# facebookresearch/DetectAndTrack

Measured on AMD Instinct MI355X. Metric: clips/sec (8-frame 800px), higher is better.
Workload: dtype bf16; 1 GPU; 3D R-18 FPN3D keypoint R-CNN inference, 4 clip(s) of 1x3x8x768x1344 per step (= per forward) per GPU (kT=3 body+FPN, slice-center 2D heads, per clip: 1000 proposals, 100 detections -> kps_score -> decoded keypoints); mode=infer, weights=random-init (synthetic_params, seed 3), images_per_forward=4, forwards_in_flight=3, clips_in_flight=12, keyframe_dce=False, hip_graph=True, resident_input=True, parallelism=clip-sharded x1 (no data-path collective)

## Files before the change

### detectandtrack_amd/csrc/conv_special.hip

```cpp
#include "conv_internal.h"

using namespace dat_conv;

namespace {

struct Ws64Params {
    const char* x;
    const char* w;
    const float* scale;
    const float* bias;
    const char* res;
    char* y;
    const char* zeros;
    int frames, H, W, out_cs, relu, res_mode;
    int tiles_h, tiles_w, ntiles;
    int ablate;
};

template <int TWL>
__global__ __launch_bounds__(NTHREADS) __attribute__((amdgpu_waves_per_eu(1, 1))) void conv3x3_c64_ws_kernel(const Ws64Params p) {
    constexpr int TW = 1 << TWL, TH = 256 >> TWL, PW = TW + 2, PH = TH + 2;
    constexpr int NPIX = PH * PW, NPIECE = (NPIX * 8 + 63) / 64, PBYTES = NPIECE * 1024, UMAX = (NPIECE + 3) / 4;
    extern __shared__ __attribute__((aligned(16))) char smem[];
    const int tid = threadIdx.x, lane = tid & 63;
// ... 598 lines not shown
__global__ __launch_bounds__(KS_THREADS) void conv_kt1x1_ks_kernel(const TkParams p) {
    constexpr int CB = 256;
    constexpr int NWQ = CB / 64;
    constexpr int NJ = NWQ;
    constexpr int WBYTES = CB / 32 * 4 * 1024;
    constexpr int WPIECES = CB / 64;
    extern __shared__ __attribute__((aligned(16))) char smem[];
    char* const xb = smem;
    char* const wb = smem + 3 * KS_XBYTES;
    const int tid = threadIdx.x, lane = tid & 63;
    const int wave = __builtin_amdgcn_readfirstlane(tid >> 6);
    const int khalf = lane >> 5, n = lane & 31;
    unsigned bid = blockIdx.x;
    if (p.xcd) bid = xcd_block_map(bid, gridDim.x);
    const int cb = bid % p.ncb;
    const unsigned pos0 = (bid / p.ncb) * 256u;
    const int wq = wave % NWQ, ph = wave / NWQ;
    typedef const __attribute__((address_space(1))) void* gptr_t;
    typedef __attribute__((address_space(3))) void* lptr_t;
    const char* xsrc[4];
    int tq[4];
#pragma unroll
    for (int u = 0; u < 4; ++u) {
        const int row = wave * 32 + u * 8 + (lane >> 3);
        const int slot = (lane & 7) ^ ((row >> 1) & 7);
        const unsigned pos = min(pos0 + (unsigned)row, p.npos - 1u);
        const unsigned f = pos / p.how;
        tq[u] = (int)(f % (unsigned)p.T);
        xsrc[u] = p.x + (size_t)pos * (unsigned)p.in_cs * 2u + slot * 16;
    }
    const char* wsrc = p.w + (size_t)cb * (CB / 32) * 4096 + (size_t)(wave * WPIECES) * 1024 + lane * 16;
    const size_t wstep = (size_t)p.mb_total * 4096;
    const ptrdiff_t fstep = (ptrdiff_t)p.how * p.in_cs * 2;
    char* const xdma = xb + wave * (32 * 128);
    char* const wdma = wb + wave * (WPIECES * 1024);
    int rq_t = 0, rq_c = 0;
#define TK_DMA_X(BUF_)                                                                                       \
    {                                                                                                        \
        const int kt_ = min(rq_t, p.kt_n - 1), cc_ = rq_t < p.kt_n ? rq_c : p.ncc - 1;                       \
        const int dt_ = kt_ - p.pt;                                                                          \
        const ptrdiff_t off_ = (ptrdiff_t)dt_ * fstep + cc_ * 128;                                           \
        _Pragma("unroll") for (int u_ = 0; u_ < 4; ++u_) {                                                   \
            const bool in_ = (unsigned)(tq[u_] + dt_) < (unsigned)p.T;                                       \
            const char* s_ = in_ ? xsrc[u_] + off_ : p.zeros;                                     \
            __builtin_amdgcn_global_load_lds((gptr_t)s_, (lptr_t)(xdma + (BUF_) * KS_XBYTES + u_ * 1024), 16, 0, 0); \
        }                                                                                                    \
        if (++rq_c == p.ncc) { rq_c = 0; ++rq_t; }                                                           \
    }
#define TK_DMA_W(KC_, BUF_)                                                                                  \
    {                                                                                                        \
        const char* ws_ = wsrc + (size_t)min((KC_), p.kchunks - 1) * wstep;                                  \
        _Pragma("unroll") for (int u_ = 0; u_ < WPIECES; ++u_)                                               \
            __builtin_amdgcn_global_load_lds((gptr_t)(ws_ + u_ * 1024), (lptr_t)(wdma + (BUF_) * WBYTES + u_ * 1024), 16, 0, 0); \
    }
#define TK_COMPUTE(XBUF_, WBUF_)                                                                             \
    {                                                                                                        \
        const char* xc_ = xb + (XBUF_) * KS_XBYTES + b_base;                                                 \
        const char* wc_ = wb + (WBUF_) * WBYTES + a_off;                                                     \
        _Pragma("unroll") for (int ks_ = 0; ks_ < 4; ++ks_) {                                                \
            uint4 a_[2], b_[NJ];                                                                             \
            _Pragma("unroll") for (int i_ = 0; i_ < 2; ++i_) a_[i_] = *(const uint4*)(wc_ + (i_ * 4 + ks_) * 1024); \
            _Pragma("unroll") for (int j_ = 0; j_ < NJ; ++j_) b_[j_] = *(const uint4*)(xc_ + j_ * 4096 + b_slot[ks_]); \
            _Pragma("unroll") for (int i_ = 0; i_ < 2; ++i_)                                                 \
                _Pragma("unroll") for (int j_ = 0; j_ < NJ; ++j_) Mma<DAT_BF16>::step(a_[i_], b_[j_], acc[i_][j_]); \
        }                                                                                                    \
    }
    TK_DMA_W(0, 0);
    TK_DMA_X(0);
    TK_DMA_X(1);
    f32x16_t acc[2][NJ];
#pragma unroll
    for (int i = 0; i < 2; ++i)
#pragma unroll
        for (int j = 0; j < NJ; ++j)
#pragma unroll
            for (int r = 0; r < 16; ++r) acc[i][j][r] = 0.f;
    const int a_off = (2 * wq) * 4096 + lane * 16;
    const int b_base = (ph * (32 * NJ) + n) * 128;
    int b_slot[4];
#pragma unroll
    for (int ks = 0; ks < 4; ++ks) b_slot[ks] = (((ks * 2 + khalf) ^ (n >> 1)) & 7) << 4;
    asm volatile("s_waitcnt vmcnt(4)" ::: "memory");
    __syncthreads();
    int xi = 0;
    for (int kc = 0; kc < p.kchunks; ++kc) {
        const int x2 = xi >= 1 ? xi - 1 : 2;
        TK_DMA_W(kc + 1, (kc + 1) & 1);
        TK_DMA_X(x2);
        TK_COMPUTE(xi, kc & 1);
        asm volatile("s_waitcnt vmcnt(4)" ::: "memory");
        __syncthreads();
        xi = xi == 2 ? 0 : xi + 1;
    }
    asm volatile("s_waitcnt vmcnt(0)" ::: "memory");
    __syncthreads();
#undef TK_DMA_X
#undef TK_DMA_W
#undef TK_COMPUTE
    char* const est = smem + wave * (32 * EPI_PITCH);
    const int sq = lane & 7, spl = lane >> 3;
    const int c0 = cb * CB + wq * 64 + sq * 8;
    float sc[8], bi[8];
#pragma unroll
    for (int e = 0; e < 8; ++e) {
        const bool ok = c0 + e < p.cout;
        const int c = ok ? c0 + e : 0;
        sc[e] = ok ? (p.scale ? p.scale[c] : 1.f) : 0.f;
        bi[e] = (ok && p.bias) ? p.bias[c] : 0.f;
    }
    const unsigned cres = (unsigned)min(c0, p.out_cs - 8);
#pragma unroll
    for (int j = 0; j < NJ; ++j) {
        const unsigned tile0 = pos0 + (unsigned)(ph * (32 * NJ) + j * 32);
        uint4 rr[4];
        if (p.res_mode) {
#pragma unroll
            for (int r = 0; r < 4; ++r) {
                const unsigned pc = min(tile0 + (unsigned)(r * 8 + spl), p.npos - 1u);
                rr[r] = *(const uint4*)(p.res + ((size_t)pc * (unsigned)p.out_cs + cres) * 2u);
            }
        }
#pragma unroll
        for (int i = 0; i < 2; ++i) epi_stage(est, n, khalf, i, acc[i][j]);
        __builtin_amdgcn_wave_barrier();
#pragma unroll
        for (int r = 0; r < 4; ++r) {
            const int pl = r * 8 + spl;
            float v[8];
            epi_load(est, pl, sq * 8, v);
            epi_affine(v, sc, bi);
            if (p.res_mode) epi_residual<DAT_BF16>(v, rr[r], 1);
            epi_relu(v, p.relu);
            const unsigned pos = tile0 + (unsigned)pl;
            if (pos < p.npos && c0 < p.cout)
                epi_store<DAT_BF16>(p.y + ((size_t)pos * (unsigned)p.out_cs + (unsigned)c0) * 2u, v);
        }
        __builtin_amdgcn_wave_barrier();
    }
}

template <int TWL, int R, int MF>
__global__ __launch_bounds__(NTHREADS) __attribute__((amdgpu_waves_per_eu(1, 1))) void conv3x3_bt_kernel(const ConvParams p) {
    constexpr int TW = 1 << TWL, TH = 256 >> TWL, PW = TW + 2, PH = TH + 2;
    constexpr int NPIX = PH * PW, NPIECE = (NPIX * 8 + 63) / 64, PBYTES = NPIECE * 1024, UMAX = (NPIECE + 3) / 4;
    constexpr int NSTEP = MF ? 18 : 36, APS = MF ? 8 : 4;
    static_assert(NSTEP % R == 0 && PBYTES < 65536, "ring slots are static per unrolled step; 16-bit patch addresses");
    static_assert(APS * R + UMAX < 64, "vmcnt is a 6-bit counter");
    typedef unsigned u32x4_t __attribute__((ext_vector_type(4)));
    typedef const __attribute__((address_space(1))) void* gptr_t;
    typedef __attribute__((address_space(3))) void* lptr_t;
    extern __shared__ __attribute__((aligned(16))) char smem[];
    unsigned long long clk_c0 = 0, clk_r0 = 0;
    if (p.clk) { clk_c0 = __builtin_amdgcn_s_memtime(); clk_r0 = __builtin_amdgcn_s_memrealtime(); }
    const int tid = threadIdx.x, lane = tid & 63;
    const int wave = __builtin_amdgcn_readfirstlane(tid >> 6);
    const int wave_n = wave & 1, wave_p = wave >> 1;
    const int khalf = lane >> 5, n = lane & 31;

    const unsigned bid = xcd_block_map(blockIdx.x, p.nblocks);
    const int nb = bid % p.nblk_n;
    unsigned tile = bid / p.nblk_n;
    const int fc = tile % p.otn; tile /= p.otn;
    const int tw_i = tile % p.tiles_w; tile /= p.tiles_w;
    const int th_i = tile % p.tiles_h;
    const int clip = tile / p.tiles_h;
    const int f = clip * p.otn + fc;
    const int t = p.ot0 + fc;
    const int f_in = clip * p.T + t;
    const int oh0 = th_i * TH, ow0 = tw_i * TW;

    int kt_lo = 0, kt_hi = p.KT - 1;
    while (kt_lo < p.KT && (t + kt_lo - p.pt) < p.in_lo) ++kt_lo;
    while (kt_hi >= 0 && (t + kt_hi - p.pt) >= p.in_hi) --kt_hi;
    const int n_kt = kt_hi - kt_lo + 1;
    const int npat = n_kt * p.n_cchunks;
    const int kt_hi_x = kt_lo + n_kt;
    int kshift = 0;
    if (n_kt == p.KT && (DAT_KT_ROTATE)) kshift = (p.KT - (t + kt_lo - p.pt) % p.KT) % p.KT;
    int kt = kt_lo + kshift, cc = 0;
    if (kt >= kt_hi_x) kt -= n_kt;

    constexpr int NJ = MF ? 8 : 4;
    unsigned qp[9][NJ / 2];
#pragma unroll
    for (int tp = 0; tp < 9; ++tp)
#pragma unroll
        for (int j = 0; j < NJ; ++j) {
            const int pos = wave_p * 128 + (MF ? j * 16 + (lane & 15) : j * 32 + n);
            const int r = pos >> TWL, c = pos & (TW - 1);
            const int row = (r + tp / 3) * PW + c + tp % 3;
            const unsigned a16 = patch_frag_addr<MF>(row, MF ? lane >> 4 : khalf);
            if (j & 1) qp[tp][j >> 1] |= a16 << 16; else qp[tp][j >> 1] = a16;
        }
    const size_t wd_cc_stride = (size_t)(p.Cout_pad >> 5) * 4096;
    const size_t tap_stride = (size_t)p.n_cchunks * wd_cc_stride;
    const char* const wd_base = p.w + (size_t)(nb * 8 + wave_n * 4) * 4096;
    unsigned aoff[APS];
#pragma unroll
    for (int i = 0; i < APS; ++i) {
        if (MF) {
            const unsigned kg = (unsigned)lane >> 4;
            aoff[i] = 16u * ((unsigned)((i & 1) << 4) + ((unsigned)lane & 15u) + 32u * (kg & 1u)) + (kg >> 1) * 1024u + (unsigned)(i >> 1) * 4096u;
        } else {
            aoff[i] = (unsigned)lane * 16u + (unsigned)i * 4096u;
        }
    }

#define BT_DMA(KT_, CC_, B_)                                                                                              \
    {                                                                                                                     \
        const int fin_ = f_in + (KT_) - p.pt;                                                                             \
        const char* xf_ = p.x + ((size_t)fin_ * p.H * p.W) * p.Cin * 2 + (size_t)(CC_) * 128;                             \
        _Pragma("unroll") for (int u_ = 0; u_ < UMAX; ++u_) {                                                             \
            const int piece_ = min(wave + 4 * u_, NPIECE - 1);                                                            \
            const int it_ = piece_ * 64 + lane, row_ = it_ >> 3;                                                          \
            const int slot_ = patch_src_slot<MF>(it_);                                                                    \
            const int prow_ = row_ / PW, pcol_ = row_ - prow_ * PW;                                                       \
            const int ih_ = oh0 - 1 + prow_, iw_ = ow0 - 1 + pcol_;                                                       \
            const bool ok_ = row_ < NPIX && (unsigned)ih_ < (unsigned)p.H && (unsigned)iw_ < (unsigned)p.W;               \
            const char* src_ = ok_ ? xf_ + ((size_t)(unsigned)(ih_ * p.W + iw_) * (unsigned)(p.Cin * 2) + (unsigned)(slot_ * 16)) : p.zeros; \
            __builtin_amdgcn_global_load_lds((gptr_t)src_, (lptr_t)(smem + (B_) * PBYTES + piece_ * 1024), 16, 0, 0);     \
        }                                                                                                                 \
    }
#define BT_WPATCH(KT_, CC_) (wd_base + ((size_t)((KT_) * 9) * p.n_cchunks + (CC_)) * wd_cc_stride)
    constexpr int SPT = NSTEP / 9;
#define BT_ALOAD(WP_, S_, SLOT_)                                                                                          \
    {                                                                                                                     \
        const char* wt_ = (WP_) + (size_t)((S_) / SPT) * tap_stride;                                                      \
        _Pragma("unroll") for (int i_ = 0; i_ < APS; ++i_)                                                                \
            asm volatile("global_load_dwordx4 %0, %1, %2 offset:%3" : "=v"(aq[SLOT_][i_]) : "v"(aoff[i_]), "s"(wt_), "n"(((S_) % SPT) * (4096 / SPT)) : "memory"); \
    }
#define BT_BREAD(U_, BOFF_)                                                                                               \
    {                                                                                                                     \
        if ((U_) % 4 == 0) {                                                                                              \
            unsigned q0_ = qp[(U_) / 4][0], q1_ = qp[(U_) / 4][1], q2_ = qp[(U_) / 4][NJ / 2 - 2], q3_ = qp[(U_) / 4][NJ / 2 - 1]; \
            asm volatile("" : "+v"(q0_), "+v"(q1_));    \
            ba[0] = (q0_ & 0xffffu) + (BOFF_); ba[1] = (q0_ >> 16) + (BOFF_);                                             \
            ba[2] = (q1_ & 0xffffu) + (BOFF_); ba[3] = (q1_ >> 16) + (BOFF_);                                             \
            if constexpr (MF != 0) {                                                                                      \
                asm volatile("" : "+v"(q2_), "+v"(q3_));                                                                  \
                ba[NJ - 4] = (q2_ & 0xffffu) + (BOFF_); ba[NJ - 3] = (q2_ >> 16) + (BOFF_);                               \
                ba[NJ - 2] = (q3_ & 0xffffu) + (BOFF_); ba[NJ - 1] = (q3_ >> 16) + (BOFF_);                               \
            }                                                                                                             \
        }                                                                                                                 \
        _Pragma("unroll") for (int j_ = 0; j_ < 4; ++j_)                                                                  \
            asm volatile("ds_read_b128 %0, %1" : "=v"(bq[(U_) % 2][j_])                                                   \
                         : "v"(ba[(MF ? ((U_) % 2) * 4 : 0) + j_] ^ (unsigned)(MF ? (((U_) / 2) % 2) << 6 : ((U_) % 4) << 5)) : "memory"); \
    }
#define BT_MFMA(ACC_, A_, B_)                                                                                             \
    {                                                                                                                     \
        if constexpr (MF) asm volatile(DAT_MFMA16K32_OP " %0, %1, %2, %0" : "+a"(ACC_) : "v"(A_), "v"(B_) : "memory");    \
        else asm volatile(DAT_MFMA16_OP " %0, %1, %2, %0" : "+a"(ACC_) : "v"(A_), "v"(B_) : "memory");                    \
    }

    typedef std::conditional_t<MF != 0, f32x4_t, f32x16_t> acc_t;
    acc_t acc[APS][NJ];
#pragma unroll
    for (int i = 0; i < APS; ++i)
#pragma unroll
        for (int j = 0; j < NJ; ++j)
#pragma unroll
            for (int r = 0; r < (MF ? 4 : 16); ++r) acc[i][j][r] = 0.f;
    u32x4_t aq[R][APS], bq[2][4];
    unsigned ba[NJ] = {};

    if (npat > 0) {
        BT_DMA(kt, cc, 0);
        const char* wcur = BT_WPATCH(kt, cc);
        static_for(std::make_integer_sequence<int, R>{}, [&](auto ic_) __attribute__((always_inline)) {
            constexpr int s0 = decltype(ic_)::value;
            (void)&aq; (void)&aoff;
            BT_ALOAD(wcur, s0, s0);
        });
        asm volatile("s_waitcnt vmcnt(%0)" :: "n"(APS * R) : "memory");
        __syncthreads();
        int buf = 0;
        for (int pi = 0; pi < npat; ++pi, buf ^= 1) {
            int ncc = cc + 1, nkt = kt;
            if (ncc == p.n_cchunks) { ncc = 0; if (++nkt == kt_hi_x) nkt = kt_lo; }
            const bool has_next = pi + 1 < npat;
            if (has_next) BT_DMA(nkt, ncc, buf ^ 1);
            const char* wnxt = has_next ? BT_WPATCH(nkt, ncc) : wcur;
            const unsigned boff = (unsigned)buf * PBYTES;
            __builtin_amdgcn_s_setprio(1);
            BT_BREAD(0, boff);
            static_for(std::make_integer_sequence<int, 36>{}, [&](auto ic_) __attribute__((always_inline)) {
                constexpr int un = decltype(ic_)::value;
                constexpr int st = MF ? un / 2 : un, jb = MF ? (un % 2) * 4 : 0;
                constexpr bool opens = !MF || un % 2 == 0, ends = !MF || un % 2 == 1;
                (void)&aq; (void)&aoff; (void)&bq; (void)&ba; (void)&acc; (void)&qp;
                if (un + 1 < 36) BT_BREAD(un + 1, boff);
                if (un + 1 < 36) asm volatile("s_waitcnt lgkmcnt(4)" ::: "memory"); else asm volatile("s_waitcnt lgkmcnt(0)" ::: "memory");
                if constexpr (opens) {
                    if constexpr (st < R) {
                        if (has_next) asm volatile("s_waitcnt vmcnt(%0)" :: "n"(APS * (R - 1) + UMAX) : "memory");
                        else asm volatile("s_waitcnt vmcnt(%0)" :: "n"(APS * (R - 1)) : "memory");
                    } else {
                        asm volatile("s_waitcnt vmcnt(%0)" :: "n"(APS * (R - 1)) : "memory");
                    }
                }
#pragma unroll
                for (int i = 0; i < APS; ++i)
#pragma unroll
                    for (int j = 0; j < 4; ++j) BT_MFMA(acc[i][jb + j], aq[st % R][i], bq[un % 2][j]);
                if constexpr (ends) {
                    if constexpr (st + R < NSTEP) { BT_ALOAD(wcur, st + R, st % R); } else { BT_ALOAD(wnxt, st + R - NSTEP, st % R); }
                }
            });
            __builtin_amdgcn_s_setprio(0);
            __syncthreads();
            kt = nkt; cc = ncc; wcur = wnxt;
        }
    }
    asm volatile("s_waitcnt vmcnt(0) lgkmcnt(0)\n\ts_nop 15\n\ts_nop 15" ::: "memory");
#undef BT_MFMA
#undef BT_BREAD
#undef BT_ALOAD
#undef BT_WPATCH
#undef BT_DMA

    constexpr int EPITCH = EPI_PITCH;
    char* const est = smem + wave * (32 * EPITCH);
    const int sl_c = (lane & 7) * 8, sl_p = lane >> 3;
    const size_t tile_pos = ((size_t)f * p.Ho + oh0) * p.Wo + ow0;
    char* const ybase = p.y + tile_pos * p.out_cs * 2;
    const char* const rbase = p.res_mode == 2 ? p.res + (size_t)f * (p.Ho >> 1) * (p.Wo >> 1) * p.out_cs * 2 : p.res + tile_pos * p.out_cs * 2;
#pragma unroll
    for (int h = 0; h < 2; ++h) {
        const int c_st = nb * 256 + wave_n * 128 + h * 64 + sl_c;
        float sc[8], bi[8];
#pragma unroll
        for (int e = 0; e < 8; ++e) {
            const bool ok = (c_st + e) < p.Cout;
            sc[e] = (p.scale && ok) ? p.scale[c_st + e] : 1.f;
            bi[e] = (p.bias && ok) ? p.bias[c_st + e] : 0.f;
        }
        uint4 rq[2][4];
        const bool res_on = p.res_mode && c_st < p.Cout;
        auto res_fetch = [&](int j, uint4* dst) __attribute__((always_inline)) {
#pragma unroll
            for (int q = 0; q < 4; ++q) {
                const int pl = q * 8 + sl_p;
                const int ohl = TWL == 5 ? 4 * wave_p + j : 8 * wave_p + 2 * j + (pl >> 4), owl = TWL == 5 ? pl : (pl & 15);
                const int oh = oh0 + ohl, ow = ow0 + owl;
                const bool live = oh < p.Ho && ow < p.Wo && !(p.ablate & 4);
                unsigned rpos = (unsigned)(ohl * p.Wo + owl);
                if (p.res_mode == 2) rpos = (unsigned)((oh >> 1) * (p.Wo >> 1) + (ow >> 1));
                dst[q] = *(const uint4*)(rbase + (live ? (rpos * (unsigned)p.out_cs + (unsigned)c_st) * 2u : 0u));
            }
        };
        if (res_on) res_fetch(0, rq[0]);
#pragma unroll
        for (int j = 0; j < 4; ++j) {
            if (res_on && j + 1 < 4) res_fetch(j + 1, rq[(j + 1) & 1]);
            if constexpr (MF) {
#pragma unroll
                for (int i = 0; i < 4; ++i)
#pragma unroll
                    for (int jl = 0; jl < 2; ++jl) epi_stage16(est, lane, i, jl, acc[(4 * h + i) % APS][(2 * j + jl) % NJ]);
            } else {
#pragma unroll
                for (int i = 0; i < 2; ++i)
#pragma unroll
                    for (int g = 0; g < 4; ++g)
                        *(float4*)(est + n * EPITCH + (i * 32 + g * 8 + khalf * 4) * 4) =
                            make_float4(acc[2 * h + i][j][g * 4 + 0], acc[2 * h + i][j][g * 4 + 1], acc[2 * h + i][j][g * 4 + 2], acc[2 * h + i][j][g * 4 + 3]);
            }
            __builtin_amdgcn_wave_barrier();
#pragma unroll
            for (int q = 0; q < 4; ++q) {
                const int pl = q * 8 + sl_p;
                const float4 t0 = *(const float4*)(est + pl * EPITCH + sl_c * 4);
                const float4 t1 = *(const float4*)(est + pl * EPITCH + sl_c * 4 + 16);
                float v[8] = {t0.x, t0.y, t0.z, t0.w, t1.x, t1.y, t1.z, t1.w};
                const int ohl = TWL == 5 ? 4 * wave_p + j : 8 * wave_p + 2 * j + (pl >> 4), owl = TWL == 5 ? pl : (pl & 15);
                const int oh = oh0 + ohl, ow = ow0 + owl;
                if (oh >= p.Ho || ow >= p.Wo || c_st >= p.Cout || (p.ablate & 4)) continue;
                const unsigned lpos = (unsigned)(ohl * p.Wo + owl);
#pragma unroll
                for (int e = 0; e < 8; ++e) v[e] = v[e] * sc[e] + bi[e];
                if (p.res_mode) {
                    const uint4 r = rq[j & 1][q];
                    const uint32_t ru[4] = {r.x, r.y, r.z, r.w};
#pragma unroll
                    for (int e2 = 0; e2 < 4; ++e2) {
                        v[2 * e2] += bf2f((uint16_t)(ru[e2] & 0xffff));
                        v[2 * e2 + 1] += bf2f((uint16_t)(ru[e2] >> 16));
                    }
                }
                if (p.relu) {
#pragma unroll
                    for (int e = 0; e < 8; ++e) v[e] = fmaxf(v[e], 0.f);
                }
                *(uint4*)(ybase + (lpos * (unsigned)p.out_cs + (unsigned)c_st) * 2u) =
                    make_uint4(f2bf2(v[0], v[1]), f2bf2(v[2], v[3]), f2bf2(v[4], v[5]), f2bf2(v[6], v[7]));
            }
            __builtin_amdgcn_wave_barrier();
        }
    }
    if (p.clk && threadIdx.x == 0) {
        atomicAdd(&p.clk[0], __builtin_amdgcn_s_memtime() - clk_c0);
        atomicAdd(&p.clk[1], __builtin_amdgcn_s_memrealtime() - clk_r0);
    }
}

}

namespace dat_conv {

bool ws64_eligible(const dat_ctx* ctx, const dat_conv_desc* d) {
    return ctx->dbg_ws64 && d->dtype == DAT_BF16 && d->Cin == 64 && d->Cout == 64 && d->KT == 1 && d->KH == 3 && d->KW == 3 &&
           d->stride_h == 1 && d->stride_w == 1 && d->pad_h == 1 && d->pad_w == 1 && d->pad_t == 0 && d->res_mode != 2 &&
           d->out_tn <= 0 && d->out_cstride % 8 == 0 && conv_dilation(d) == 1;
}

int ctx_num_cu(dat_ctx* ctx);
static long long persist_cus(dat_ctx* ctx, int mult) {
    long long n = ctx_num_cu(ctx);
    if (ctx->dbg_persist_pct > 0 && ctx->dbg_persist_pct < 100) n = std::max<long long>(mult, n * ctx->dbg_persist_pct / 100 / mult * mult);
    return n;
}

int ctx_num_cu(dat_ctx* ctx) {
    if (ctx->num_cu == 0) {
        int dev = 0, n = 0;
        if (hipGetDevice(&dev) != hipSuccess || hipDeviceGetAttribute(&n, hipDeviceAttributeMultiprocessorCount, dev) != hipSuccess) n = 0;
        ctx->num_cu = n > 0 ? n : 256;
    }
    return ctx->num_cu;
}

bool bt_eligible(const dat_ctx* ctx, const dat_conv_desc* d) {
    return ctx->dbg_bt && d->dtype == DAT_BF16 && d->Cin % 64 == 0 && cout_pad_of(d) % 256 == 0 && d->Cout % 8 == 0 && d->KH == 3 && d->KW == 3 &&
           d->stride_h == 1 && d->stride_w == 1 && d->pad_h == 1 && d->pad_w == 1 && d->out_cstride % 8 == 0 && conv_dilation(d) == 1;
}

int bt_tile_twl(const ConvParams& p, long long* nblocks) {
    int best = 4;
    long long best_tiles = -1;
    for (int twl = 4; twl <= 5; ++twl) {
        const long long tiles = cdiv_ll(p.Ho, 256 >> twl) * cdiv_ll(p.Wo, 1 << twl);
        if (best_tiles < 0 || tiles < best_tiles) { best_tiles = tiles; best = twl; }
    }
    *nblocks = best_tiles * p.frames * (p.Cout_pad / 256);
    return best;
}

int launch_bt(dat_ctx* ctx, hipStream_t st, ConvParams& p) {
    long long nblocks = 0;
    const int twl = bt_tile_twl(p, &nblocks);
    const int tw = 1 << twl, th = 256 >> twl;
    p.th_log2 = 8 - twl; p.tw_log2 = twl; p.tile_w = tw;
    p.tiles_h = (int)cdiv_ll(p.Ho, th); p.tiles_w = (int)cdiv_ll(p.Wo, tw);
    p.n_cchunks = p.Cin / 64;
    p.nblk_n = p.Cout_pad / 256;
    p.ksplit = 1; p.part = nullptr;
    p.ablate = ctx->dbg_ablate;
    DAT_ENFORCE(ctx, nblocks > 0 && nblocks < (1ll << 31), "conv3d: grid of %lld blocks unsupported", nblocks);
    DAT_ENFORCE(ctx, (long long)p.Ho * p.Wo * std::max(p.out_cs, p.Cout) * 4 < (1ll << 31) && (long long)p.H * p.W * p.Cin * 2 < (1ll << 32),
                "conv3d: one frame of %dx%d exceeds the 32-bit offsets of the big-tile kernel", p.H, p.W);
    p.nblocks = (unsigned)nblocks;
    const int npiece = ((th + 2) * (tw + 2) * 8 + 63) / 64;
    const size_t lds = (size_t)2 * npiece * 1024;
#define BT_LAUNCH(TWL_, R_, MF_)                                                                                           \
    {                                                                                                                  \
        if (dat_ensure_lds(ctx, (const void*)conv3x3_bt_kernel<TWL_, R_, MF_>, 160 * 1024) != DAT_OK) return DAT_ERR_LAUNCH; \
        hipLaunchKernelGGL((conv3x3_bt_kernel<TWL_, R_, MF_>), dim3(p.nblocks), dim3(NTHREADS), lds, st, p);           \
    }
    if (ctx->dbg_mfma) { if (twl == 5) BT_LAUNCH(5, 3, 1) else BT_LAUNCH(4, 3, 1) }
    else if (twl == 5) BT_LAUNCH(5, 6, 0) else BT_LAUNCH(4, 6, 0)
#undef BT_LAUNCH
    DAT_CHECK_LAUNCH(ctx, "conv3x3_bt");
    return DAT_OK;
}

bool pw256_eligible(const dat_ctx* ctx, const dat_conv_desc* d) {
    return ctx->dbg_ws64 && d->dtype == DAT_BF16 && d->Cin == 64 && d->Cout == 256 && d->KT == 1 && d->KH == 1 && d->KW == 1 &&
           d->stride_h == 1 && d->stride_w == 1 && d->pad_h == 0 && d->pad_w == 0 && d->pad_t == 0 && d->out_tn <= 0 &&
           d->out_cstride % 8 == 0 &&
           (long long)d->H * d->W >= 32 && (long long)d->H * d->W * d->W < (1ll << 32) &&
           (long long)d->frames * d->H * d->W * std::max(d->out_cstride, 64) * 2 < (1ll << 32);
}

int launch_pw256(dat_ctx* ctx, hipStream_t st, const ConvParams& cp) {
    Pw256Params p;
    p.x = cp.x; p.w = cp.w; p.scale = cp.scale; p.bias = cp.bias; p.res = cp.res; p.y = cp.y;
    p.npos = (long long)cp.frames * cp.H * cp.W;
    p.H = cp.H; p.W = cp.W; p.out_cs = cp.out_cs; p.relu = cp.relu; p.res_mode = cp.res_mode;
    const long long ntiles = cdiv_ll(p.npos, 32);
    DAT_ENFORCE(ctx, ntiles > 0 && ntiles < (1ll << 31), "conv3d: %lld wave tiles unsupported", ntiles);
    p.ntiles = (int)ntiles;
    p.hw = (unsigned)(cp.H * cp.W);
    p.w_magic = cp.W == 1 ? 0u : (unsigned)((0x100000000ull + (unsigned)cp.W - 1) / (unsigned)cp.W);
    const unsigned grid = (unsigned)std::min<long long>(cdiv_ll(ntiles, 4), persist_cus(ctx, 8));
    const size_t lds = (size_t)4 * 32 * (256 * 4 + 16);
    if (dat_ensure_lds(ctx, (const void*)conv1x1_k64_c256_ws_kernel, 160 * 1024) != DAT_OK) return DAT_ERR_LAUNCH;
    hipLaunchKernelGGL(conv1x1_k64_c256_ws_kernel, dim3(grid), dim3(NTHREADS), lds, st, p);
    DAT_CHECK_LAUNCH(ctx, "conv1x1_k64_c256_ws");
    return DAT_OK;
}

static int lw_nsplit(const dat_conv_desc* d) {
    const long long wbytes = (long long)d->Cin * cout_pad_of(d) * 2;
    int ns = 1;
    while (wbytes / ns > 128 * 1024) ns *= 2;
    return ns;
}

bool pwlw_eligible(dat_ctx* ctx, const dat_conv_desc* d) {
    if (!(ctx->dbg_pwlw && d->dtype == DAT_BF16 && d->KT == 1 && d->KH == 1 && d->KW == 1 && d->pad_h == 0 && d->pad_w == 0 && d->pad_t == 0 &&
          d->out_tn <= 0 && d->stride_h == d->stride_w && (d->stride_h == 1 || d->stride_h == 2)))
        return false;
    const int kc = d->Cin / 64;
    if (d->Cin % 64 || !(kc == 1 || kc == 2 || kc == 4 || kc == 8)) return false;
    const int ns = lw_nsplit(d), mbt = cout_pad_of(d) / 32;
    if (ns > 4 || mbt % ns) return false;
    const int mbp = mbt / ns;
    if (!(mbp == 2 || mbp == 4 || mbp == 8 || mbp == 16) || (kc == 8 && mbp > 4)) return false;
    if ((long long)kc * mbp * 4096 + mbp * 256 + 4 * 32 * 144 > 160 * 1024) return false;
    if (d->out_cstride % 8 || d->out_cstride < d->Cout) return false;
    int Ho, Wo;
    dat_conv3d_out_shape(d, &Ho, &Wo);
    const long long npos = (long long)d->frames * Ho * Wo;
    if ((long long)Ho * Wo < 32 || (long long)Ho * Wo * Wo >= (1ll << 32)) return false;
    if (npos >= (1ll << 31) || (long long)d->frames * d->H * d->W >= (1ll << 31)) return false;
    return npos / 32 >= 2ll * 4 * ctx_num_cu(ctx) / ns;
}

template <int KC, int MBW, int NPASS>
static int launch_pwlw_t(dat_ctx* ctx, hipStream_t st, const PwLwParams& p, unsigned grid, size_t lds) {
    if (p.res_mode == 4) {
        if (dat_ensure_lds(ctx, (const void*)conv1x1_lw_kernel<KC, MBW, NPASS, 1>, 160 * 1024) != DAT_OK) return DAT_ERR_LAUNCH;
        hipLaunchKernelGGL((conv1x1_lw_kernel<KC, MBW, NPASS, 1>), dim3(grid), dim3(NTHREADS), lds, st, p);
        return DAT_OK;
    }
    if (dat_ensure_lds(ctx, (const void*)conv1x1_lw_kernel<KC, MBW, NPASS>, 160 * 1024) != DAT_OK) return DAT_ERR_LAUNCH;
    hipLaunchKernelGGL((conv1x1_lw_kernel<KC, MBW, NPASS>), dim3(grid), dim3(NTHREADS), lds, st, p);
    return DAT_OK;
}

int launch_pwlw(dat_ctx* ctx, hipStream_t st, const ConvParams& cp, const dat_conv_desc* d) {
    PwLwParams p;
    p.x = cp.x; p.w = cp.w; p.scale = cp.scale; p.bias = cp.bias; p.res = cp.res; p.y = cp.y; p.res2 = cp.res2;
    p.npos = (unsigned)((long long)cp.frames * cp.Ho * cp.Wo);
    p.Ho = cp.Ho; p.Wo = cp.Wo; p.H = cp.H; p.W = cp.W; p.stride = cp.sh;
    p.in_cs = cp.Cin; p.out_cs = cp.out_cs; p.cout = cp.Cout; p.relu = cp.relu; p.res_mode = cp.res_mode;
    p.ntiles = (int)cdiv_ll(p.npos, 32);
    p.how = (unsigned)(cp.Ho * cp.Wo);
    p.wo_magic = cp.Wo == 1 ? 0u : (unsigned)((0x100000000ull + (unsigned)cp.Wo - 1) / (unsigned)cp.Wo);
    p.nsplit = lw_nsplit(d); p.mb_total = cp.Cout_pad / 32;
    const int kc = cp.Cin / 64, mbp = p.mb_total / p.nsplit;
    const int mbw = kc <= 4 ? std::min(mbp, 8) : std::min(mbp, 4), npass = mbp / mbw;
    const long long per_part = std::min<long long>(cdiv_ll(p.ntiles, 4), persist_cus(ctx, 8 * p.nsplit) / p.nsplit);
    const unsigned grid = (unsigned)(per_part * p.nsplit);
    p.xcd = ctx->dbg_pw_xcd && p.nsplit > 1 && grid % (8u * (unsigned)p.nsplit) == 0;
    const size_t lds = (size_t)kc * mbp * 4096 + (size_t)mbp * 32 * 8 + 4 * 32 * (32 * 4 + 16);
    DAT_ENFORCE(ctx, lds <= 160 * 1024, "conv1x1_lw: %zu bytes of LDS", lds);
    int rc = DAT_ERR_UNSUPPORTED;
#define LW_CASE(KC_, MBW_, NP_) if (kc == KC_ && mbw == MBW_ && npass == NP_) rc = launch_pwlw_t<KC_, MBW_, NP_>(ctx, st, p, grid, lds);
    LW_CASE(1, 2, 1) LW_CASE(1, 4, 1) LW_CASE(1, 8, 1) LW_CASE(1, 8, 2)
    LW_CASE(2, 2, 1) LW_CASE(2, 4, 1) LW_CASE(2, 8, 1) LW_CASE(2, 8, 2)
    LW_CASE(4, 2, 1) LW_CASE(4, 4, 1) LW_CASE(4, 8, 1)
    LW_CASE(8, 2, 1) LW_CASE(8, 4, 1)
#undef LW_CASE
    if (rc != DAT_OK) DAT_FAIL(ctx, rc, "conv1x1_lw: no instantiation for K chunks %d x %d row blocks x %d passes", kc, mbw, npass);
    DAT_CHECK_LAUNCH(ctx, "conv1x1_lw");
    return DAT_OK;
}

bool pwks_eligible(dat_ctx* ctx, const dat_conv_desc* d) {
    if (!(ctx->dbg_pwks > 0 && d->dtype == DAT_BF16 && d->KT == 1 && d->KH == 1 && d->KW == 1 && d->pad_h == 0 && d->pad_w == 0 && d->pad_t == 0 &&
          d->out_tn <= 0 && d->stride_h == d->stride_w && (d->stride_h == 1 || d->stride_h == 2)))
        return false;
    if (d->Cin % 64 || d->Cin / 64 < ctx->dbg_pwks || cout_pad_of(d) % 256) return false;
    if (d->out_cstride % 8 || d->out_cstride < d->Cout || d->out_cstride < 8) return false;
    int Ho, Wo;
    dat_conv3d_out_shape(d, &Ho, &Wo);
    const long long npos = (long long)d->frames * Ho * Wo;
    if ((long long)Ho * Wo < 1 || (long long)Ho * Wo * Wo >= (1ll << 32)) return false;
    if (npos >= (1ll << 31) || (long long)d->frames * d->H * d->W >= (1ll << 31)) return false;
    const long long blocks = cdiv_ll(npos, 256) * (cout_pad_of(d) / 256);
    return npos >= 256 && blocks * 4 >= 3ll * ctx_num_cu(ctx);
}

int launch_pwks(dat_ctx* ctx, hipStream_t st, const ConvParams& cp) {
    PwKsParams p;
    p.x = cp.x; p.w = cp.w; p.scale = cp.scale; p.bias = cp.bias; p.res = cp.res; p.y = cp.y; p.res2 = cp.res2;
    p.npos = (unsigned)((long long)cp.frames * cp.Ho * cp.Wo);
    p.Ho = cp.Ho; p.Wo = cp.Wo; p.H = cp.H; p.W = cp.W; p.stride = cp.sh;
    p.in_cs = cp.Cin; p.out_cs = cp.out_cs; p.cout = cp.Cout; p.relu = cp.relu; p.res_mode = cp.res_mode;
    p.ncb = cp.Cout_pad / 256; p.kchunks = cp.Cin / 64; p.mb_total = cp.Cout_pad / 32;
    p.how = (unsigned)(cp.Ho * cp.Wo);
    p.wo_magic = cp.Wo == 1 ? 0u : (unsigned)((0x100000000ull + (unsigned)cp.Wo - 1) / (unsigned)cp.Wo);
    p.ablate = ctx->dbg_ablate;
    p.xcd = ctx->dbg_pw_xcd && p.ncb > 1;
    const long long blocks = cdiv_ll(p.npos, 256) * p.ncb;
    DAT_ENFORCE(ctx, blocks > 0 && blocks < (1ll << 31), "conv1x1_ks: grid of %lld blocks unsupported", blocks);
    const size_t lds = (size_t)3 * KS_XBYTES + 2 * KS_WBYTES;
    if (dat_ensure_lds(ctx, (const void*)conv1x1_ks_kernel, 160 * 1024) != DAT_OK) return DAT_ERR_LAUNCH;
    hipLaunchKernelGGL(conv1x1_ks_kernel, dim3((unsigned)blocks), dim3(KS_THREADS), lds, st, p);
    DAT_CHECK_LAUNCH(ctx, "conv1x1_ks");
    return DAT_OK;
}

bool tks_eligible(dat_ctx* ctx, const dat_conv_desc* d) {
    if (!(ctx->dbg_temporal > 0 && DAT_H16_FORMAT == 0 && d->dtype == DAT_BF16 && d->KT > 1 && d->KH == 1 && d->KW == 1 && d->pad_h == 0 &&
          d->pad_w == 0 && d->pad_t * 2 + 1 == d->KT && d->out_tn <= 0 && d->in_tn <= 0 && d->stride_h == 1 && d->stride_w == 1 &&
          (d->res_mode == 0 || d->res_mode == 1)))
        return false;
    if (d->Cin % 64 || cout_pad_of(d) % 256) return false;
    if (d->out_cstride % 8 || d->out_cstride < d->Cout || d->out_cstride < 8) return false;
    const long long how = (long long)d->H * d->W, npos = (long long)d->frames * how;
    if (how < 1 || npos >= (1ll << 31) || npos * d->Cin >= (1ll << 40)) return false;
    const long long blocks = cdiv_ll(npos, 256) * (cout_pad_of(d) / 256);
    return npos >= 256 && (ctx->dbg_temporal >= 2 || blocks * 4 >= 3ll * ctx_num_cu(ctx));
}

int launch_tks(dat_ctx* ctx, hipStream_t st, const ConvParams& cp) {
    TkParams p;
    p.x = cp.x; p.w = cp.w; p.scale = cp.scale; p.bias = cp.bias; p.res = cp.res; p.zeros = cp.zeros; p.y = cp.y;
    p.npos = (unsigned)((long long)cp.frames * cp.Ho * cp.Wo);
    p.how = (unsigned)(cp.Ho * cp.Wo);
    p.T = cp.T; p.pt = cp.pt; p.kt_n = cp.KT;
    p.in_cs = cp.Cin; p.out_cs = cp.out_cs; p.cout = cp.Cout; p.relu = cp.relu; p.res_mode = cp.res_mode;
// ... 48 lines not shown
```

Baseline: 276.1 clips/s.

## Prefetch scale/bias to LDS and double-buffer the big-tile conv epilogue

```diff
diff --git a/detectandtrack_amd/csrc/conv_special.hip b/detectandtrack_amd/csrc/conv_special.hip
--- a/detectandtrack_amd/csrc/conv_special.hip
+++ b/detectandtrack_amd/csrc/conv_special.hip
@@ -774,6 +774,19 @@
     extern __shared__ __attribute__((aligned(16))) char smem[];
     unsigned long long clk_c0 = 0, clk_r0 = 0;
     if (p.clk) { clk_c0 = __builtin_amdgcn_s_memtime(); clk_r0 = __builtin_amdgcn_s_memrealtime(); }
+#ifdef DAT_CONV_TRACE
+#define BT_STAMP(T_)                                                                          \
+    {                                                                                         \
+        __builtin_amdgcn_sched_barrier(0);                                                    \
+        asm volatile("s_memtime %0\n\ts_waitcnt lgkmcnt(0)" : "=s"(T_) :: "memory");          \
+        __builtin_amdgcn_sched_barrier(0);                                                    \
+    }
+    unsigned long long tr_k0 = 0, tr_first = 0, tr_k1 = 0, tr_st = 0, tr_end = 0;
+    BT_STAMP(tr_k0);
+    tr_first = tr_k0;
+#else
+#define BT_STAMP(T_)
+#endif
     const int tid = threadIdx.x, lane = tid & 63;
     const int wave = __builtin_amdgcn_readfirstlane(tid >> 6);
     const int wave_n = wave & 1, wave_p = wave >> 1;
@@ -803,17 +816,7 @@
     if (kt >= kt_hi_x) kt -= n_kt;
 
     constexpr int NJ = MF ? 8 : 4;
-    unsigned qp[9][NJ / 2];
-#pragma unroll
-    for (int tp = 0; tp < 9; ++tp)
-#pragma unroll
-        for (int j = 0; j < NJ; ++j) {
-            const int pos = wave_p * 128 + (MF ? j * 16 + (lane & 15) : j * 32 + n);
-            const int r = pos >> TWL, c = pos & (TW - 1);
-            const int row = (r + tp / 3) * PW + c + tp % 3;
-            const unsigned a16 = patch_frag_addr<MF>(row, MF ? lane >> 4 : khalf);
-            if (j & 1) qp[tp][j >> 1] |= a16 << 16; else qp[tp][j >> 1] = a16;
-        }
+    constexpr int SB_OFF = 2 * PBYTES;
     const size_t wd_cc_stride = (size_t)(p.Cout_pad >> 5) * 4096;
     const size_t tap_stride = (size_t)p.n_cchunks * wd_cc_stride;
     const char* const wd_base = p.w + (size_t)(nb * 8 + wave_n * 4) * 4096;
@@ -875,26 +878,55 @@
     }
 
     typedef std::conditional_t<MF != 0, f32x4_t, f32x16_t> acc_t;
-    acc_t acc[APS][NJ];
-#pragma unroll
-    for (int i = 0; i < APS; ++i)
-#pragma unroll
-        for (int j = 0; j < NJ; ++j)
-#pragma unroll
-            for (int r = 0; r < (MF ? 4 : 16); ++r) acc[i][j][r] = 0.f;
     u32x4_t aq[R][APS], bq[2][4];
     unsigned ba[NJ] = {};
 
+    {
+        const int c = nb * 256 + wave * 64 + lane;
+        const bool ok = c < p.Cout;
+        const char* const ssrc = (p.scale && ok) ? (const char*)(p.scale + c) : p.zeros;
+        const char* const bsrc = (p.bias && ok) ? (const char*)(p.bias + c) : p.zeros;
+        __builtin_amdgcn_global_load_lds((gptr_t)ssrc, (lptr_t)(smem + SB_OFF + wave * 256), 4, 0, 0);
+        __builtin_amdgcn_global_load_lds((gptr_t)bsrc, (lptr_t)(smem + SB_OFF + 1024 + wave * 256), 4, 0, 0);
+    }
+    const char* wcur = nullptr;
     if (npat > 0) {
         BT_DMA(kt, cc, 0);
-        const char* wcur = BT_WPATCH(kt, cc);
+        wcur = BT_WPATCH(kt, cc);
         static_for(std::make_integer_sequence<int, R>{}, [&](auto ic_) __attribute__((always_inline)) {
             constexpr int s0 = decltype(ic_)::value;
             (void)&aq; (void)&aoff;
             BT_ALOAD(wcur, s0, s0);
         });
+    }
+    __builtin_amdgcn_sched_barrier(0);
+
+    unsigned qp[9][NJ / 2];
+#pragma unroll
+    for (int tp = 0; tp < 9; ++tp)
+#pragma unroll
+        for (int j = 0; j < NJ; ++j) {
+            const int pos = wave_p * 128 + (MF ? j * 16 + (lane & 15) : j * 32 + n);
+            const int r = pos >> TWL, c = pos & (TW - 1);
+            const int row = (r + tp / 3) * PW + c + tp % 3;
+            const unsigned a16 = patch_frag_addr<MF>(row, MF ? lane >> 4 : khalf);
+            if (j & 1) qp[tp][j >> 1] |= a16 << 16; else qp[tp][j >> 1] = a16;
+        }
+    acc_t acc[APS][NJ];
+#pragma unroll
+    for (int i = 0; i < APS; ++i)
+#pragma unroll
+        for (int j = 0; j < NJ; ++j)
+#pragma unroll
+            for (int r = 0; r < (MF ? 4 : 16); ++r) acc[i][j][r] = 0.f;
+
+    if (npat <= 0) {
+        asm volatile("s_waitcnt vmcnt(0)" ::: "memory");
+        __syncthreads();
+    } else {
         asm volatile("s_waitcnt vmcnt(%0)" :: "n"(APS * R) : "memory");
         __syncthreads();
+        BT_STAMP(tr_first);
         int buf = 0;
         for (int pi = 0; pi < npat; ++pi, buf ^= 1) {
             int ncc = cc + 1, nkt = kt;
@@ -934,91 +966,144 @@
         }
     }
     asm volatile("s_waitcnt vmcnt(0) lgkmcnt(0)\n\ts_nop 15\n\ts_nop 15" ::: "memory");
+    BT_STAMP(tr_k1);
 #undef BT_MFMA
 #undef BT_BREAD
 #undef BT_ALOAD
 #undef BT_WPATCH
 #undef BT_DMA
 
-    constexpr int EPITCH = EPI_PITCH;
-    char* const est = smem + wave * (32 * EPITCH);
+    constexpr int EPITCH = EPI_PITCH, ESLICE = 32 * EPITCH;
+    static_assert(4 * 2 * ESLICE <= 2 * PBYTES, "the staging slices live in the two patch buffers");
+    char* const est = smem + wave * (2 * ESLICE);
     const int sl_c = (lane & 7) * 8, sl_p = lane >> 3;
     const size_t tile_pos = ((size_t)f * p.Ho + oh0) * p.Wo + ow0;
     char* const ybase = p.y + tile_pos * p.out_cs * 2;
     const char* const rbase = p.res_mode == 2 ? p.res + (size_t)f * (p.Ho >> 1) * (p.Wo >> 1) * p.out_cs * 2 : p.res + tile_pos * p.out_cs * 2;
+#define BT_PIN(X_) asm volatile("" : "+s"(X_))
+    int relu = p.relu, res_mode = p.res_mode, wo2 = p.Wo >> 1, out_cs = p.out_cs;
+    unsigned row_b = (unsigned)p.Wo * (unsigned)p.out_cs * 2u, col8_b = (unsigned)p.out_cs * 16u;
+    BT_PIN(relu); BT_PIN(res_mode); BT_PIN(wo2); BT_PIN(out_cs); BT_PIN(row_b); BT_PIN(col8_b);
+#undef BT_PIN
+    const int ohl0 = (TWL == 5 ? 4 : 8) * wave_p, c0 = nb * 256 + wave_n * 128 + sl_c;
+    const unsigned off0 = ((unsigned)(ohl0 * p.Wo + sl_p) * (unsigned)p.out_cs + (unsigned)c0) * 2u;
+    unsigned lmask = 0;
+#pragma unroll
+    for (int jq = 0; jq < 16; ++jq) {
+        const int drow = TWL == 5 ? jq >> 2 : 2 * (jq >> 2) + ((jq & 3) >> 1), dcol8 = TWL == 5 ? jq & 3 : jq & 1;
+        if (oh0 + ohl0 + drow < p.Ho && ow0 + sl_p + 8 * dcol8 < p.Wo && !(p.ablate & 4)) lmask |= 1u << jq;
+    }
+    const unsigned lmask_h[2] = {c0 < p.Cout ? lmask : 0u, c0 + 64 < p.Cout ? lmask : 0u};
+    float sc[2][8], bi[2][8];
 #pragma unroll
     for (int h = 0; h < 2; ++h) {
-        const int c_st = nb * 256 + wave_n * 128 + h * 64 + sl_c;
-        float sc[8], bi[8];
+        const int cl = wave_n * 128 + h * 64 + sl_c;
+        const bool ok = nb * 256 + cl < p.Cout;
+        const float4 s0 = *(const float4*)(smem + SB_OFF + cl * 4), s1 = *(const float4*)(smem + SB_OFF + cl * 4 + 16);
+        const float4 b0 = *(const float4*)(smem + SB_OFF + 1024 + cl * 4), b1 = *(const float4*)(smem + SB_OFF + 1024 + cl * 4 + 16);
+        const float sv[8] = {s0.x, s0.y, s0.z, s0.w, s1.x, s1.y, s1.z, s1.w}, bv[8] = {b0.x, b0.y, b0.z, b0.w, b1.x, b1.y, b1.z, b1.w};
 #pragma unroll
         for (int e = 0; e < 8; ++e) {
-            const bool ok = (c_st + e) < p.Cout;
-            sc[e] = (p.scale && ok) ? p.scale[c_st + e] : 1.f;
-            bi[e] = (p.bias && ok) ? p.bias[c_st + e] : 0.f;
-        }
-        uint4 rq[2][4];
-        const bool res_on = p.res_mode && c_st < p.Cout;
-        auto res_fetch = [&](int j, uint4* dst) __attribute__((always_inline)) {
+            sc[h][e] = (p.scale && ok) ? sv[e] : 1.f;
+            bi[h][e] = (p.bias && ok) ? bv[e] : 0.f;
+        }
+    }
+    auto row_live = [&](int rd, int q) __attribute__((always_inline)) { return (lmask_h[rd >> 2] >> ((rd & 3) * 4 + q)) & 1u; };
+    auto row_off = [&](int rd, int q) __attribute__((always_inline)) {
+        const int jq = (rd & 3) * 4 + q;
+        const int drow = TWL == 5 ? jq >> 2 : 2 * (jq >> 2) + ((jq & 3) >> 1), dcol8 = TWL == 5 ? jq & 3 : jq & 1;
+        return off0 + (unsigned)drow * row_b + (unsigned)dcol8 * col8_b + (unsigned)(rd >> 2) * 128u;
+    };
+    uint4 rq[2][4];
+    auto res_fetch = [&](int rd, uint4* dst) __attribute__((always_inline)) {
+#pragma unroll
+        for (int q = 0; q < 4; ++q) {
+            unsigned roff = row_off(rd, q);
+            if (res_mode == 2) {
+                const int jq = (rd & 3) * 4 + q;
+                const int drow = TWL == 5 ? jq >> 2 : 2 * (jq >> 2) + ((jq & 3) >> 1), dcol8 = TWL == 5 ? jq & 3 : jq & 1;
+                const unsigned rpos = (unsigned)(((oh0 + ohl0 + drow) >> 1) * wo2 + ((ow0 + sl_p + 8 * dcol8) >> 1));
+                roff = (rpos * (unsigned)out_cs + (unsigned)(c0 + (rd >> 2) * 64)) * 2u;
+            }
+            dst[q] = *(const uint4*)(rbase + (row_live(rd, q) ? roff : 0u));
+        }
+    };
+    auto stage = [&](auto rd_) __attribute__((always_inline)) {
+        constexpr int rd = decltype(rd_)::value, h = rd >> 2, j = rd & 3;
+        char* const es = est + (rd & 1) * ESLICE;
+        (void)&acc;
+        if constexpr (MF != 0) {
+#pragma unroll
+            for (int i = 0; i < 4; ++i)
+#pragma unroll
+                for (int jl = 0; jl < 2; ++jl) epi_stage16(es, lane, i, jl, acc[(4 * h + i) % APS][(2 * j + jl) % NJ]);
+        } else {
+#pragma unroll
+            for (int i = 0; i < 2; ++i)
+#pragma unroll
+                for (int g = 0; g < 4; ++g)
+                    *(float4*)(es + n * EPITCH + (i * 32 + g * 8 + khalf * 4) * 4) =
+                        make_float4(acc[2 * h + i][j][g * 4 + 0], acc[2 * h + i][j][g * 4 + 1], acc[2 * h + i][j][g * 4 + 2], acc[2 * h + i][j][g * 4 + 3]);
+        }
+    };
+    if (res_mode) res_fetch(0, rq[0]);
+    stage(std::integral_constant<int, 0>{});
+    static_for(std::make_integer_sequence<int, 8>{}, [&](auto rd_) __attribute__((always_inline)) {
+        constexpr int rd = decltype(rd_)::value, h = rd >> 2;
+        (void)&acc; (void)&sc; (void)&bi; (void)&rq;
+        __builtin_amdgcn_wave_barrier();
+        if (res_mode && rd + 1 < 8) res_fetch(rd + 1, rq[(rd + 1) & 1]);
+        const char* const es = est + (rd & 1) * ESLICE;
+        float v[4][8];
+#pragma unroll
+        for (int q = 0; q < 4; ++q) {
+            const int pl = q * 8 + sl_p;
+            const float4 t0 = *(const float4*)(es + pl * EPITCH + sl_c * 4);
+            const float4 t1 = *(const float4*)(es + pl * EPITCH + sl_c * 4 + 16);
+            v[q][0] = t0.x; v[q][1] = t0.y; v[q][2] = t0.z; v[q][3] = t0.w; v[q][4] = t1.x; v[q][5] = t1.y; v[q][6] = t1.z; v[q][7] = t1.w;
+        }
+        if constexpr (rd + 1 < 8) stage(std::integral_constant<int, rd + 1>{});
+#pragma unroll
+        for (int q = 0; q < 4; ++q)
+#pragma unroll
+            for (int e = 0; e < 8; ++e) v[q][e] = v[q][e] * sc[h][e] + bi[h][e];
+        if (res_mode) {
 #pragma unroll
             for (int q = 0; q < 4; ++q) {
-                const int pl = q * 8 + sl_p;
-                const int ohl = TWL == 5 ? 4 * wave_p + j : 8 * wave_p + 2 * j + (pl >> 4), owl = TWL == 5 ? pl : (pl & 15);
-                const int oh = oh0 + ohl, ow = ow0 + owl;
-                const bool live = oh < p.Ho && ow < p.Wo && !(p.ablate & 4);
-                unsigned rpos = (unsigned)(ohl * p.Wo + owl);
-                if (p.res_mode == 2) rpos = (unsigned)((oh >> 1) * (p.Wo >> 1) + (ow >> 1));
-                dst[q] = *(const uint4*)(rbase + (live ? (rpos * (unsigned)p.out_cs + (unsigned)c_st) * 2u : 0u));
+                const uint4 r = rq[rd & 1][q];
+                const uint32_t ru[4] = {r.x, r.y, r.z, r.w};
+#pragma unroll
+                for (int e2 = 0; e2 < 4; ++e2) {
+                    v[q][2 * e2] += bf2f((uint16_t)(ru[e2] & 0xffff));
+                    v[q][2 * e2 + 1] += bf2f((uint16_t)(ru[e2] >> 16));
+                }
             }
-        };
-        if (res_on) res_fetch(0, rq[0]);
-#pragma unroll
-        for (int j = 0; j < 4; ++j) {
-            if (res_on && j + 1 < 4) res_fetch(j + 1, rq[(j + 1) & 1]);
-            if constexpr (MF) {
-#pragma unroll
-                for (int i = 0; i < 4; ++i)
-#pragma unroll
-                    for (int jl = 0; jl < 2; ++jl) epi_stage16(est, lane, i, jl, acc[(4 * h + i) % APS][(2 * j + jl) % NJ]);
-            } else {
-#pragma unroll
-                for (int i = 0; i < 2; ++i)
-#pragma unroll
-                    for (int g = 0; g < 4; ++g)
-                        *(float4*)(est + n * EPITCH + (i * 32 + g * 8 + khalf * 4) * 4) =
-                            make_float4(acc[2 * h + i][j][g * 4 + 0], acc[2 * h + i][j][g * 4 + 1], acc[2 * h + i][j][g * 4 + 2], acc[2 * h + i][j][g * 4 + 3]);
-            }
-            __builtin_amdgcn_wave_barrier();
-#pragma unroll
-            for (int q = 0; q < 4; ++q) {
-                const int pl = q * 8 + sl_p;
-                const float4 t0 = *(const float4*)(est + pl * EPITCH + sl_c * 4);
-                const float4 t1 = *(const float4*)(est + pl * EPITCH + sl_c * 4 + 16);
-                float v[8] = {t0.x, t0.y, t0.z, t0.w, t1.x, t1.y, t1.z, t1.w};
-                const int ohl = TWL == 5 ? 4 * wave_p + j : 8 * wave_p + 2 * j + (pl >> 4), owl = TWL == 5 ? pl : (pl & 15);
-                const int oh = oh0 + ohl, ow = ow0 + owl;
-                if (oh >= p.Ho || ow >= p.Wo || c_st >= p.Cout || (p.ablate & 4)) continue;
-                const unsigned lpos = (unsigned)(ohl * p.Wo + owl);
-#pragma unroll
-                for (int e = 0; e < 8; ++e) v[e] = v[e] * sc[e] + bi[e];
-                if (p.res_mode) {
-                    const uint4 r = rq[j & 1][q];
-                    const uint32_t ru[4] = {r.x, r.y, r.z, r.w};
-#pragma unroll
-                    for (int e2 = 0; e2 < 4; ++e2) {
-                        v[2 * e2] += bf2f((uint16_t)(ru[e2] & 0xffff));
-                        v[2 * e2 + 1] += bf2f((uint16_t)(ru[e2] >> 16));
-                    }
-                }
-                if (p.relu) {
-#pragma unroll
-                    for (int e = 0; e < 8; ++e) v[e] = fmaxf(v[e], 0.f);
-                }
-                *(uint4*)(ybase + (lpos * (unsigned)p.out_cs + (unsigned)c_st) * 2u) =
-                    make_uint4(f2bf2(v[0], v[1]), f2bf2(v[2], v[3]), f2bf2(v[4], v[5]), f2bf2(v[6], v[7]));
-            }
-            __builtin_amdgcn_wave_barrier();
-        }
-    }
+        }
+        if (relu) {
+#pragma unroll
+            for (int q = 0; q < 4; ++q)
+#pragma unroll
+                for (int e = 0; e < 8; ++e) v[q][e] = fmaxf(v[q][e], 0.f);
+        }
+#pragma unroll
+        for (int q = 0; q < 4; ++q) {
+            const uint4 o = make_uint4(f2bf2(v[q][0], v[q][1]), f2bf2(v[q][2], v[q][3]), f2bf2(v[q][4], v[q][5]), f2bf2(v[q][6], v[q][7]));
+            if (row_live(rd, q)) *(uint4*)(ybase + row_off(rd, q)) = o;
+        }
+    });
+    BT_STAMP(tr_st);
+#ifdef DAT_CONV_TRACE
+    asm volatile("s_waitcnt vmcnt(0)" ::: "memory");
+    BT_STAMP(tr_end);
+    if (tid == 0 && p.dbg) {
+        atomicAdd(&p.dbg[8], tr_end - tr_k0);
+        atomicAdd(&p.dbg[9], tr_end - tr_k1);
+        atomicAdd(&p.dbg[10], tr_first - tr_k0);
+        atomicAdd(&p.dbg[11], tr_end - tr_st);
+        atomicAdd(&p.dbg[13], 1ull);
+    }
+#endif
+#undef BT_STAMP
     if (p.clk && threadIdx.x == 0) {
         atomicAdd(&p.clk[0], __builtin_amdgcn_s_memtime() - clk_c0);
         atomicAdd(&p.clk[1], __builtin_amdgcn_s_memrealtime() - clk_r0);
@@ -1082,15 +1167,31 @@
                 "conv3d: one frame of %dx%d exceeds the 32-bit offsets of the big-tile kernel", p.H, p.W);
     p.nblocks = (unsigned)nblocks;
     const int npiece = ((th + 2) * (tw + 2) * 8 + 63) / 64;
-    const size_t lds = (size_t)2 * npiece * 1024;
+    const size_t lds = (size_t)2 * npiece * 1024 + 2048;
 #define BT_LAUNCH(TWL_, R_, MF_)                                                                                           \
     {                                                                                                                  \
         if (dat_ensure_lds(ctx, (const void*)conv3x3_bt_kernel<TWL_, R_, MF_>, 160 * 1024) != DAT_OK) return DAT_ERR_LAUNCH; \
         hipLaunchKernelGGL((conv3x3_bt_kernel<TWL_, R_, MF_>), dim3(p.nblocks), dim3(NTHREADS), lds, st, p);           \
     }
+#ifdef DAT_CONV_TRACE
+    static unsigned long long* dbg = nullptr;
+    if (!dbg) hipMalloc(&dbg, 128);
+    hipMemsetAsync(dbg, 0, 128, st);
+    p.dbg = dbg;
+#endif
     if (ctx->dbg_mfma) { if (twl == 5) BT_LAUNCH(5, 3, 1) else BT_LAUNCH(4, 3, 1) }
     else if (twl == 5) BT_LAUNCH(5, 6, 0) else BT_LAUNCH(4, 6, 0)
 #undef BT_LAUNCH
+#ifdef DAT_CONV_TRACE
+    {
+        unsigned long long h[16];
+        hipStreamSynchronize(st);
+        hipMemcpy(h, dbg, 128, hipMemcpyDeviceToHost);
+        if (h[13]) fprintf(stderr, "TRACE big-tile %dx%d MF=%d blocks=%llu | per block, shader cycles: total %.0f = prologue %.0f + taps %.0f + epilogue %.0f + store drain %.0f\n",
+                           th, tw, ctx->dbg_mfma ? 1 : 0, h[13], (double)h[8] / h[13], (double)h[10] / h[13], (double)(h[8] - h[9] - h[10]) / h[13],
+                           (double)(h[9] - h[11]) / h[13], (double)h[11] / h[13]);
+    }
+#endif
     DAT_CHECK_LAUNCH(ctx, "conv3x3_bt");
     return DAT_OK;
 }
```

After: 277.8 clips/s (median of 6 runs). No clear change (+0.6%).
